# OSLL/slam-constructor

Hardware: AMD Instinct MI355X
Metric: pose-candidates*beams/sec (1080-beam scan, 2000^2 grid) (higher is better)
Workload: dtype f64; 1 GPU; cfg2: tinySLAM HC(dt 0.1, dr 0.1, failed-rounds 128), 1080 beams, 2000x2000 @0.05 m, occupancy cell; parallelism=1 gpu, ranks=1, includes_filter_and_upload=True, mode=default (canonical tree sum, device sincos; com~

## Files before the change

slam-constructor_amd/csrc/hc_chain.h:

```cpp
#pragma once

#include <cstdint>

#if defined(__HIPCC__)
#include <hip/hip_runtime.h>
#define HC_HD __host__ __device__ __forceinline__
#else
#define HC_HD inline
#endif

namespace slamhip {

constexpr int kHcMaxInst = 64;
constexpr int kHcDefaultInst = 42;
constexpr int kHcMaxSeg = 14;
constexpr int kHcShapes = 8;
constexpr int kHcSlots = 6 * kHcMaxInst + 1;

HC_HD double hc_bucket_rate(int b) { return 0.5 / (double)(1 << (kHcShapes - 1 - b)); }
HC_HD int hc_bucket_of_ratio(double num, double den) {
  int b = 0;
  for (int j = 0; j < kHcShapes - 1; ++j) b += (num > hc_bucket_rate(j) * 1.4142135623730951 * den) ? 1 : 0;
  return b;
}
HC_HD int hc_bucket_of(double p) { return hc_bucket_of_ratio(p, 1.0); }

struct HcInst {
  unsigned long long w[16];
};
static_assert(sizeof(HcInst) == 128, "HcInst layout");

HC_HD int hc_child(const HcInst &i, int out) {
  const unsigned long long v = out < 4 ? i.w[7] : i.w[8];
  return (int)(short)(unsigned short)(v >> (16 * (out & 3)));
}
HC_HD int hc_bp_inst(const HcInst &i) { return (int)(short)(unsigned short)(i.w[8] >> 48); }
HC_HD int hc_byte9(const HcInst &i, int k) { return (int)((i.w[9] >> (8 * k)) & 0xffull); }
HC_HD int hc_bp_cand(const HcInst &i) { return hc_byte9(i, 0); }
HC_HD unsigned hc_nfail(const HcInst &i) { return (unsigned)hc_byte9(i, 1); }
HC_HD unsigned hc_nfail_parent(const HcInst &i) { return (unsigned)hc_byte9(i, 2); }
HC_HD int hc_depth(const HcInst &i) { return hc_byte9(i, 3); }
HC_HD int hc_nseg(const HcInst &i) { return hc_byte9(i, 4); }
HC_HD bool hc_is_root(const HcInst &i) { return hc_byte9(i, 5) != 0; }
HC_HD unsigned hc_tail_fail(const HcInst &i) { return (unsigned)hc_byte9(i, 6); }
HC_HD int hc_parent(const HcInst &i) { return hc_byte9(i, 7) == 255 ? -1 : hc_byte9(i, 7); }
HC_HD unsigned hc_seg_fail(const HcInst &i, int k) {
  return (unsigned)(((k < 8 ? i.w[10] : i.w[11]) >> (8 * (k & 7))) & 0xffull);
}
HC_HD int hc_seg_out(const HcInst &i, int k) {
  return (int)(((k < 8 ? i.w[12] : i.w[13]) >> (8 * (k & 7))) & 0xffull);
}
inline void hc_set16(unsigned long long &w, int slot, int v) {
  w = (w & ~(0xffffull << (16 * slot))) | ((unsigned long long)(unsigned short)(short)v << (16 * slot));
}
inline void hc_set8(unsigned long long &w, int slot, unsigned v) {
  w = (w & ~(0xffull << (8 * slot))) | ((unsigned long long)(v & 0xff) << (8 * slot));
}
inline void hc_set_child(HcInst &i, int out, int v) { hc_set16(out < 4 ? i.w[7] : i.w[8], out & 3, v); }
inline void hc_set_bp_inst(HcInst &i, int v) { hc_set16(i.w[8], 3, v); }
inline void hc_set_byte9(HcInst &i, int k, unsigned v) { hc_set8(i.w[9], k, v); }
inline void hc_set_seg(HcInst &i, int k, unsigned fail, unsigned out) {
  hc_set8(k < 8 ? i.w[10] : i.w[11], k & 7, fail);
  hc_set8(k < 8 ? i.w[12] : i.w[13], k & 7, out);
}

struct HcShape {
  int n_inst;
  int pad[31];
  HcInst inst[kHcMaxInst];
};

struct HcState {
  double x, y, theta;
  double best_prob;
  double dt, dr;
  double recent_acc, recent_n;
  long long calls;
  long long evaluated;
  unsigned failed;
  int shape;
  int done;
  int first;
  int steps;
  int mode;
  int carry_cx, carry_cy;
  double carry_prob;
  unsigned long long best_hash;
  long long rescored;
};
static_assert(sizeof(HcState) == 136, "HcState layout");

HC_HD void hc_candidate(double x, double y, double theta, double dt, double dr, int c, double *ox, double *oy,
                        double *ot) {
  const double dir = (c % 2) ? -1.0 : 1.0;
  const double fcos = 1.0, fsin = 0.0;
  const int axis = c % 3;
  const double x0 = x + fcos * dir * dt, y0 = y + fsin * dir * dt;
  const double x1 = x + -fsin * dir * dt, y1 = y + fcos * dir * dt;
  const double t2 = theta + dir * dr;
  *ox = axis == 0 ? x0 : (axis == 1 ? x1 : x);
  *oy = axis == 0 ? y0 : (axis == 1 ? y1 : y);
  *ot = axis == 2 ? t2 : theta;
}

HC_HD bool hc_inert(double x, double y, double theta, double dt, double dr) {
  union U {
    double d;
    unsigned long long u;
  };
  U bx, by, bt;
  bx.d = x;
  by.d = y;
  bt.d = theta;
  bool same = true;
  for (int c = 0; c < 6; ++c) {
    U cx, cy, ct;
    hc_candidate(x, y, theta, dt, dr, c, &cx.d, &cy.d, &ct.d);
    same = same && cx.u == bx.u && cy.u == by.u && ct.u == bt.u;
  }
  return same;
}

HC_HD void hc_cert_beam(double px, double py, double sn, double cs, double theta_abs, double r_, double ca, double sa,
                        double scale, double inv_scale, double *t_t, double *t_r) {
  const double c = cs * ca - sn * sa;
  const double s_ = sn * ca + cs * sa;
  const double wx = px + r_ * c, wy = py + r_ * s_;
  const double qx = wx * inv_scale, qy = wy * inv_scale;
  const double fx = qx - __builtin_floor(qx), fy = qy - __builtin_floor(qy);
  const double mx = fx < 1.0 - fx ? fx : 1.0 - fx, my = fy < 1.0 - fy ? fy : 1.0 - fy;
  const double edge = (mx < my ? mx : my) * scale;
  const double ar = __builtin_fabs(r_);
  const double slack = (ar * (1.0 + theta_abs) + __builtin_fabs(wx) + __builtin_fabs(wy) + __builtin_fabs(px) +
                        __builtin_fabs(py) + 1.0) * 0x1p-44;
  const double avail = edge - slack;
  const bool ok = avail > 0.0;
  *t_t = ok ? avail * 0.99 : 0.0;
  *t_r = ok ? (ar > 0.0 ? avail / (1.5 * ar) : __builtin_inf()) : 0.0;
}

HC_HD double hc_pow_half(unsigned k) {
  union {
    unsigned long long u;
    double d;
  } v;
  v.u = (unsigned long long)(1023 - k) << 52;
  return v.d;
}

struct HcRound {
  double x, y, theta, dt, dr;
  unsigned failed;
};
HC_HD HcRound hc_round_of(const HcState &s, const HcInst &in) {
  HcRound r{s.x, s.y, s.theta, s.dt, s.dr, s.failed};
  const int nseg = hc_nseg(in);
  for (int k = 0; k < nseg; ++k) {
    const unsigned f = hc_seg_fail(in, k);
    const double h = hc_pow_half(f);
    r.dt *= h;
    r.dr *= h;
    r.failed += f;
    hc_candidate(r.x, r.y, r.theta, r.dt, r.dr, hc_seg_out(in, k) - 1, &r.x, &r.y, &r.theta);
  }
  const unsigned tf = hc_tail_fail(in);
  const double h = hc_pow_half(tf);
  r.dt *= h;
  r.dr *= h;
  r.failed += tf;
  return r;
}

HC_HD bool hc_trailing(unsigned failed_at_round, unsigned max_failed) { return failed_at_round >= max_failed; }

HC_HD int hc_round_outcome(double enter, const double *s, int n, double *run, int *nacc) {
  double b = enter;
  int out = 0, acc = 0;
  for (int c = 0; c < n; ++c)
    if (b < s[c]) {
      b = s[c];
      out = c + 1;
      ++acc;
    }
  *run = b;
  *nacc = acc;
  return out;
}

struct HcDecision {
  int out, nacc, last_acc;
  unsigned accmask;
  bool ambiguous;
};
HC_HD void hc_decide_one(HcDecision &d, double &b, unsigned long long &hb, int c, double s, unsigned long long h,
                         bool check) {
  union {
    double d;
    unsigned long long u;
  } sb{s}, bb{b};
  if (check && (h != hb || sb.u != bb.u)) {
    const double diff = s > b ? s - b : b - s;
    const double as = s < 0 ? -s : s, ab = b < 0 ? -b : b;
    if (diff <= (as > ab ? as : ab) * 9.094947017729282e-13) d.ambiguous = true;
  }
  if (b < s) {
    b = s;
    hb = h;
    d.out = c + 1;
    d.last_acc = c;
    d.accmask |= 1u << c;
    ++d.nacc;
  }
}
HC_HD HcDecision hc_round_decide(double enter, unsigned long long enter_hash, const double *dec,
                                 const unsigned long long *hash, int n, bool check) {
  HcDecision d{0, 0, -1, 0u, false};
  double b = enter;
  unsigned long long hb = enter_hash;
  for (int c = 0; c < n; ++c) hc_decide_one(d, b, hb, c, dec[c], hash[c], check);
  return d;
}

HC_HD HcRound hc_round_from(double x, double y, double theta, double dt, double dr, unsigned failed, const HcInst &in) {
  HcState s{};
  s.x = x;
  s.y = y;
  s.theta = theta;
  s.dt = dt;
  s.dr = dr;
  s.failed = failed;
  return hc_round_of(s, in);
}

struct HcNextCore {
  double x, y, theta, dt, dr;
  double recent_acc, recent_n;
  unsigned failed;
  int shape, done;
  long long batch_calls;
};
HC_HD HcNextCore hc_next_core(const HcState &prev, const HcInst &in, const HcRound &r, int out, unsigned max_failed) {
  HcNextCore n;
  n.x = r.x;
  n.y = r.y;
  n.theta = r.theta;
  n.dt = r.dt;
  n.dr = r.dr;
  n.failed = r.failed;
  if (out > 0) hc_candidate(r.x, r.y, r.theta, r.dt, r.dr, out - 1, &n.x, &n.y, &n.theta);
  const bool trailing = hc_trailing(r.failed, max_failed);
  n.done = trailing ? 1 : 0;
  if (!n.done && out == 0) {
    n.dt = r.dt * 0.5;
    n.dr = r.dr * 0.5;
    n.failed = r.failed + 1;
  }
  n.batch_calls = 6ll * hc_depth(in) + (trailing ? 1 : 6);
  const long long rounds_acc = (long long)hc_nseg(in) + (out > 0 ? 1 : 0);
  n.recent_acc = 0.5 * prev.recent_acc + (double)rounds_acc;
  n.recent_n = 0.5 * prev.recent_n + (double)n.batch_calls;
  n.shape = hc_bucket_of_ratio(n.recent_acc + 0.5, n.recent_n + 4.0);
  return n;
}

HC_HD void hc_advance(const HcState &prev, const HcInst &in, const HcRound &r, int out, double run, unsigned max_failed,
                      long long evaluated, HcState *next) {
  const HcNextCore c = hc_next_core(prev, in, r, out, max_failed);
  HcState n = prev;
  n.x = c.x;
  n.y = c.y;
  n.theta = c.theta;
  n.dt = c.dt;
  n.dr = c.dr;
  n.failed = c.failed;
  n.best_prob = run;
  n.done = c.done;
  n.calls = prev.calls + (prev.first ? 1 : 0) + c.batch_calls;
  n.evaluated = prev.evaluated + evaluated;
  n.first = 0;
  n.mode = 0;
  n.steps = prev.steps + 1;
  n.recent_acc = c.recent_acc;
  n.recent_n = c.recent_n;
  n.shape = c.shape;
  *next = n;
}

}
```

slam-constructor_amd/csrc/hc_resident.hip:

```cpp
#include <hip/hip_runtime.h>

#include "hc_chain_device.h"
#include "hc_resident_device.h"
#include "scan_assemble_device.h"
#include "score_device.h"

namespace slamhip {

namespace {
constexpr int kSumLanes = 256;
}

template <int H>
struct HcNextEntryT {
  double x, y, theta;
  double p[H][4];
  unsigned counts;
  unsigned flags;
};
static_assert(sizeof(HcNextEntryT<1>) == 64 && sizeof(HcNextEntryT<2>) == 96, "HcNextEntry layout");
static_assert(kHcMaxSeg + 1 <= 15, "HcNextEntry::counts: accepted rounds of a path in 4 bits");
static_assert(6 * kHcMaxInst + 6 < 4096, "HcNextEntry::counts: scorer calls of a path in 12 bits");
__device__ __forceinline__ unsigned hc_entry_counts(const HcNextCore &c, int rounds_acc) {
  return (c.failed & 0xffffu) | (((unsigned)c.batch_calls & 0xfffu) << 16) | (((unsigned)rounds_acc & 0xfu) << 28);
}

__device__ __forceinline__ void wave_min2(double &a, double &b) {
#define HCR_MIN_STEP(OFF)                              \
  {                                                    \
    const double oa = lane_xor_f64<OFF>(a), ob = lane_xor_f64<OFF>(b); \
    a = a < oa ? a : oa;                               \
    b = b < ob ? b : ob;                               \
  }
  HCR_MIN_STEP(32) HCR_MIN_STEP(16) HCR_MIN_STEP(8) HCR_MIN_STEP(4) HCR_MIN_STEP(2) HCR_MIN_STEP(1)
#undef HCR_MIN_STEP
}
__device__ __forceinline__ unsigned long long wave_xor_sum_u64(unsigned long long h) {
#define HCR_ADD_STEP(OFF)                                                                            \
  {                                                                                                  \
    const unsigned ol = lane_xor_u32<OFF>((unsigned)h), oh = lane_xor_u32<OFF>((unsigned)(h >> 32)); \
    h += ((unsigned long long)oh << 32) | ol;                                                        \
  }
  HCR_ADD_STEP(32) HCR_ADD_STEP(16) HCR_ADD_STEP(8) HCR_ADD_STEP(4) HCR_ADD_STEP(2) HCR_ADD_STEP(1)
#undef HCR_ADD_STEP
  return h;
}

constexpr int kSelRescore = -1;
constexpr int kSelFirst = -2;
constexpr int kSelStop = -3;

template <int MODEL, int NT, bool SEQ, bool BATCH, int G, bool WIN = false, bool PAIR = false, bool RAW = false>
__global__ __launch_bounds__(NT, 4) void k_hc_chain_resident(HcChainArgs a) {
  static_assert(!RAW || (!SEQ && !BATCH && !WIN && !PAIR), "RAW: the lone 1-cell chain in the default sum order only");
  constexpr int H = PAIR ? 2 : 1;
  constexpr int NTH = NT / H;
  constexpr bool CERT = !WIN;
  typedef HcNextEntryT<H> HcNextEntry;
  extern __shared__ double s_term[];
  __shared__ unsigned long long s_hash[kHcSlots + 7];
  __shared__ double s_sc[kHcSlots + 7];
  __shared__ HcInst s_mine[H][kHcShapes];
  __shared__ double s_cur[H][4];
  __shared__ int s_cur_go[H];
  __shared__ int s_sel;
  __shared__ int s_stop;
  __shared__ HcState s_st;
  __shared__ double s_part[H][4];
  __shared__ unsigned long long s_hpart[H][4];
  constexpr int kFpWaves = NTH / 64 > 4 ? NTH / 64 - 4 : 0;
  __shared__ unsigned long long s_hidle[kFpWaves > 0 ? kFpWaves : 1];
  __shared__ double s_cert[2][16];
  __shared__ int s_cert_end;
  const long long t_kernel_begin = SLAMHIP_STAMPS_ON(a.stamps != nullptr) ? (long long)wall_clock64() : 0ll;
  const int t = threadIdx.x, wave = t >> 6;
  const int half = PAIR ? (t >= NTH ? 1 : 0) : 0;
  const int tl = t - half * NTH, lwave = tl >> 6;
  const bool init_slot = blockIdx.x + 1 == gridDim.x;
  const int slot = init_slot ? kHcSlots - 1 : (PAIR ? 2 * (int)blockIdx.x + half : (int)blockIdx.x);
  const int inst_of_slot = slot / 6, cand = slot - 6 * inst_of_slot;
  const bool exists = init_slot ? half == 0 : slot < 6 * a.max_inst;
  HcResidentCtl *const rc = a.rctl + blockIdx.y;
  HcHostOut *const host = a.host + blockIdx.y;
  const unsigned fail_epoch_at_entry = __hip_atomic_load(&rc->fail_epoch, __ATOMIC_RELAXED, __HIP_MEMORY_SCOPE_AGENT);
#ifdef SLAMHIP_TESTING
  if (a.debug_mute && (int)blockIdx.x + 1 == a.debug_mute) return;
#endif
  MapViewCP map_p;
  ScanViewCP scan_p;
  {
    const __attribute__((address_space(4))) HcChainArgs *ap0 =
        (const __attribute__((address_space(4))) HcChainArgs *)__builtin_amdgcn_kernarg_segment_ptr();
    if (BATCH) {
      const __attribute__((address_space(4))) HcJobView *jv =
          (const __attribute__((address_space(4))) HcJobView *)(unsigned long long)(a.jobs + blockIdx.y);
      map_p = &jv->map;
      scan_p = &jv->scan;
    } else {
      map_p = &ap0->map;
      scan_p = &ap0->scan;
    }
  }
  const ScanView scan = load_view(scan_p);
  const int n = scan.n;
  double br = 0.0, bc = 0.0, bs = 0.0, bw = 0.0, bf = 0.0;
  if (!RAW && tl < n) {
    br = scan.range[tl];
    bc = scan.cos_a[tl];
    bs = scan.sin_a[tl];
    bw = scan.weight[tl];
    bf = scan.factor[tl];
  }
  const bool mine_here = lwave == 1 && (t & 63) < kHcShapes && !init_slot && exists;
  constexpr int kMineQ = (int)(sizeof(HcInst) / 16);
  static_assert(!RAW || kMineQ == 8, "RAW: the instance record in eight named registers");
  u32x4 mine0, mine1, mine2, mine3, mine4, mine5, mine6, mine7;
  ScanInFlight raw_first{0.0, 0.0, 0.0, 0.0, 1.0, 0}, raw_more{0.0, 0.0, 0.0, 0.0, 1.0, 0};
  HcInst first_in = {};
  const int n_last = n > 0 ? n - 1 : 0;
  const bool raw_more_wave = RAW && __builtin_amdgcn_readfirstlane(NTH + (t & ~63)) < n;
  if constexpr (RAW) {
    if (mine_here) {
      const u32x4 *src = reinterpret_cast<const u32x4 *>(&a.shapes[t & 63].inst[inst_of_slot]);
      mine0 = src[0];
      mine1 = src[1];
      mine2 = src[2];
      mine3 = src[3];
      mine4 = src[4];
      mine5 = src[5];
      mine6 = src[6];
      mine7 = src[7];
    }
    asm volatile("" ::: "memory");
    scan_assemble_issue(a.raw, tl < n ? tl : n_last, raw_first);
    if (raw_more_wave) scan_assemble_issue(a.raw, NTH + t < n ? NTH + t : n_last, raw_more);
    {
      const __attribute__((address_space(4))) HcInst *ip = (const __attribute__((address_space(4))) HcInst *)(
          unsigned long long)&a.shapes[a.shape0].inst[init_slot ? 0 : inst_of_slot];
#pragma unroll
      for (int q = 0; q < 14; ++q) first_in.w[q] = ip->w[q];
    }
  } else if (mine_here) {
    const uint4 *src = reinterpret_cast<const uint4 *>(&a.shapes[t & 63].inst[inst_of_slot]);
    uint4 *dst = reinterpret_cast<uint4 *>(&s_mine[half][t & 63]);
#pragma unroll
    for (int q = 0; q < kMineQ; ++q) dst[q] = src[q];
  }
  const bool ldsc = RAW || (!WIN && a.lds_consts != 0);
  const int n_more = n > NTH ? n - NTH : 0;
  double *const my_term = s_term + (PAIR ? half * a.scan.n : 0);
  double *const s_r = s_term + (PAIR ? 2 * a.scan.n : n) - NTH, *const s_ca = s_r + n_more, *const s_sa = s_ca + n_more;
  double *const s_w = s_sa + n_more, *const s_f = s_w + n_more;
  if (!RAW && ldsc) {
    for (int b = NTH + t; b < n; b += NT) {
      s_r[b] = scan.range[b];
      s_ca[b] = scan.cos_a[b];
      s_sa[b] = scan.sin_a[b];
    }
  }
  HcNextEntry *const s_tab = reinterpret_cast<HcNextEntry *>(s_term + a.tab_offset);
  if (!RAW && t == 0) s_stop = fail_epoch_at_entry == a.epoch ? 1 : 0;
  if (tl < 4 && exists) {
    HcGranule *g0 = (tl & 2) ? &rc->seq[tl & 1][slot] : &rc->gran[tl & 1][slot];
    gran_store(g0, 0.0, 0ull, 0u);
  }
  const bool verify = a.verify != 0;
  const bool stamp = SLAMHIP_STAMPS_ON(a.stamps && slot == 1 && tl == 0 && blockIdx.y == 0);
  [[maybe_unused]] const bool stamp_wave = SLAMHIP_STAMPS_ON(a.stamps && slot == 1 && tl < 64 && blockIdx.y == 0);
  if (stamp) a.stamps[6] = t_kernel_begin;
  HcGranule *const gran = &rc->gran[0][0];
  HcGranule *const gseq = &rc->seq[0][0];
  constexpr int kGranRow = kHcSlots + 7;

  if (t == 0) {
    HcState st{};
    const double *const inits = RAW ? nullptr : a.inits;
    st.x = inits ? inits[3 * blockIdx.y] : a.init[0];
    st.y = inits ? inits[3 * blockIdx.y + 1] : a.init[1];
    st.theta = inits ? inits[3 * blockIdx.y + 2] : a.init[2];
    st.dt = a.dt0;
    st.dr = a.dr0;
    st.shape = a.shape0;
    st.first = 1;
    st.carry_cx = st.carry_cy = -1;
    st.carry_prob = -1.0;
    s_st = st;
    s_sel = kSelFirst;
    s_cert_end = 0;
  }
  __syncthreads();
  if (!RAW && s_stop) return;
  if (lwave == 0) {
    const HcState &st = s_st;
    bool go = exists;
    double px = st.x, py = st.y, pth = st.theta;
    if (!init_slot && exists) {
      HcInst in;
#pragma unroll
      for (int q = 0; q < 14; ++q) in.w[q] = RAW ? first_in.w[q] : s_mine[half][st.shape].w[q];
      go = inst_of_slot < (int)((a.n_inst >> (8 * st.shape)) & 0xffull) &&
           (hc_is_root(in) || st.failed + hc_nfail_parent(in) < a.max_failed);
      if (go) {
        const HcRound r = hc_round_of(st, in);
        go = !(hc_trailing(r.failed, a.max_failed) && cand > 0);
        hc_candidate(r.x, r.y, r.theta, r.dt, r.dr, cand, &px, &py, &pth);
      }
    }
    double sn, cs;
    sincos(pth, &sn, &cs);
    if (tl == 0) {
      s_cur[half][0] = px;
      s_cur[half][1] = py;
      s_cur[half][2] = sn;
      s_cur[half][3] = cs;
      s_cur_go[half] = go ? 1 : 0;
    }
  }
  if constexpr (RAW) {
    const auto keep = [&](int b, const ScanPoint &p) __attribute__((always_inline)) {
      s_r[b] = p.range;
      s_ca[b] = p.cos_a;
      s_sa[b] = p.sin_a;
      s_w[b] = p.weight;
      s_f[b] = p.factor;
    };
    scan_assemble_wait(raw_first, raw_more);
    asm volatile("" ::"v"(mine0), "v"(mine1), "v"(mine2), "v"(mine3), "v"(mine4), "v"(mine5), "v"(mine6), "v"(mine7),
                 "v"(fail_epoch_at_entry));
    {
      ScanPoint p, pm;
      scan_assemble_finish(a.raw, raw_first, raw_more, p, pm);
      if (tl < n) {
        br = p.range;
        bc = p.cos_a;
        bs = p.sin_a;
        bw = p.weight;
        bf = p.factor;
      }
      if (NTH + t < n) keep(NTH + t, pm);
    }
    if (mine_here) {
      u32x4 *dst = reinterpret_cast<u32x4 *>(&s_mine[half][t & 63]);
      dst[0] = mine0;
      dst[1] = mine1;
      dst[2] = mine2;
      dst[3] = mine3;
      dst[4] = mine4;
      dst[5] = mine5;
      dst[6] = mine6;
      dst[7] = mine7;
    }
    if (t == 0) s_stop = fail_epoch_at_entry == a.epoch ? 1 : 0;
    for (int b = NTH + NT + t; b - (t & 63) < n; b += 2 * NT) {
      ScanInFlight f0{0.0, 0.0, 0.0, 0.0, 1.0, 0}, f1{0.0, 0.0, 0.0, 0.0, 1.0, 0};
      scan_assemble_issue(a.raw, b < n ? b : n_last, f0);
      scan_assemble_issue(a.raw, b + NT < n ? b + NT : n_last, f1);
      scan_assemble_wait(f0, f1);
      ScanPoint p0, p1;
      scan_assemble_finish(a.raw, f0, f1, p0, p1);
      if (b < n) keep(b, p0);
      if (b + NT < n) keep(b + NT, p1);
    }
  }
  __syncthreads();
  if (RAW && s_stop) return;

  auto write_scan_block = [&](int t, double *dst, int stride) __attribute__((always_inline)) {
    for (int q = t; q < stride; q += NT) {
      double r_ = 0.0, ca = 0.0, sa = 0.0, w = 0.0, f = 0.0;
      if (q < NT && q < n) {
        r_ = br;
        ca = bc;
        sa = bs;
        w = bw;
        f = bf;
      } else if (q < n) {
        r_ = s_r[q];
        ca = s_ca[q];
        sa = s_sa[q];
        w = s_w[q];
        f = s_f[q];
      }
      dst[q] = r_;
      dst[stride + q] = ca;
      dst[2 * stride + q] = sa;
      dst[3 * stride + q] = w;
      dst[4 * stride + q] = f;
    }
  };
  const int t_entry = t;
  for (int k = 0;; ++k) {
    const int pk = k & 1;
    int t = t_entry;
    asm volatile("" : "+v"(t));
    const int lane = t & 63;
    const int tl = PAIR ? t - half * NTH : t;
    const __attribute__((address_space(4))) HcChainArgs *ap =
        (const __attribute__((address_space(4))) HcChainArgs *)__builtin_amdgcn_kernarg_segment_ptr();
    asm volatile("" : "+s"(ap));
    MapViewCP mp = map_p;
    asm volatile("" : "+s"(mp));
    const MapView map = load_view(mp);
    if (stamp && k < 64) ap->stamps[8 * k + 0] = wall_clock64();
    const int sel = s_sel;
    if (sel == kSelStop) break;
    int go, mode = 0;
    double px, py, sn, cs;
    if (sel >= 0) {
      const HcNextEntry &e = s_tab[sel];
      const unsigned flags = e.flags;
      const bool cert_end = CERT && s_cert_end != 0;
      const int done = (int)((flags >> 3) & 1u) | (cert_end ? 1 : 0);
      go = (int)((flags >> (4 + half)) & 1u);
      px = e.p[half][0];
      py = e.p[half][1];
      sn = e.p[half][2];
      cs = e.p[half][3];
      if (wave == NT / 64 - 1 && lane < 1 + H) {
        if (lane == 0) {
          HcState &w = s_st;
          const unsigned counts = e.counts;
          const unsigned failed = counts & 0xffffu;
          const double half = hc_pow_half(failed - w.failed);
          w.x = e.x;
          w.y = e.y;
          w.theta = e.theta;
          w.dt = w.dt * half;
          w.dr = w.dr * half;
          w.recent_acc = 0.5 * w.recent_acc + (double)(counts >> 28);
          w.recent_n = 0.5 * w.recent_n + (double)((counts >> 16) & 0xfffu);
          w.failed = failed;
          w.shape = (int)(flags & 7u);
          w.done = done;
        } else {
          const int hh = lane - 1;
          s_cur[hh][0] = e.p[hh][0];
          s_cur[hh][1] = e.p[hh][1];
          s_cur[hh][2] = e.p[hh][2];
          s_cur[hh][3] = e.p[hh][3];
          s_cur_go[hh] = (int)((flags >> (4 + hh)) & 1u);
        }
      }
      long long tail_calls = 0;
      if (done && ((flags & 64u) || cert_end)) tail_calls = 6ll * (long long)(ap->max_failed - (e.counts & 0xffffu)) + 1ll;
      if (done && init_slot && tail_calls > 0 && ap->trace) {
        __syncthreads();
        HcTraceEntry *const trace = ap->trace + (size_t)blockIdx.y * (size_t)ap->trace_stride;
        const long long at0 = s_st.calls;
        const double best = s_st.best_prob, dt_e = s_st.dt, dr_e = s_st.dr;
        for (long long q = t; q < tail_calls; q += NT) {
          const double hlf = hc_pow_half((unsigned)(q / 6));
          HcTraceEntry te;
          hc_candidate(e.x, e.y, e.theta, dt_e * hlf, dr_e * hlf, (int)(q % 6), &te.x, &te.y, &te.theta);
          te.score = best;
          te.accepted = 0;
          te.pad = 0;
          if (at0 + q < ap->trace_cap) trace[at0 + q] = te;
          else host->error = 2;
        }
        __threadfence_system();
        __syncthreads();
      }
      if (done && init_slot && t == 0) {
        const HcState &w = s_st;
        const long long t_over = SLAMHIP_STAMPS_ON(ap->stamps != nullptr) ? (long long)wall_clock64() : 0ll;
        __threadfence_system();
        HcHostOut *h = host;
        h->pose[0] = e.x;
        h->pose[1] = e.y;
        h->pose[2] = e.theta;
        h->best_prob = w.best_prob;
        h->calls = w.calls + tail_calls;
        h->tail_calls = tail_calls;
        h->evaluated = w.evaluated;
        h->steps = w.steps;
        h->rescored = w.rescored;
        h->gm_cx = -1;
        h->gm_cy = -1;
        h->gm_prob = -1.0;
        __hip_atomic_store(&h->done_seq, ap->epoch, __ATOMIC_RELEASE, __HIP_MEMORY_SCOPE_SYSTEM);
        if (SLAMHIP_STAMPS_ON(ap->stamps != nullptr) && blockIdx.y == 0) {
          asm volatile("s_waitcnt vmcnt(0)" ::: "memory");
          ap->stamps[8 + 6] = t_over;
          ap->stamps[16 + 6] = wall_clock64();
        }
        if (ap->n_done) {
          __threadfence_system();
          const unsigned before = atomicAdd(ap->n_done, 1u);
          if (before + 1u == gridDim.y && ap->h_all_done)
            __hip_atomic_store(ap->h_all_done, ap->epoch, __ATOMIC_RELEASE, __HIP_MEMORY_SCOPE_SYSTEM);
        }
      }
      if constexpr (RAW) {
        if (done && init_slot && k == 1) write_scan_block(t, ap->raw.dst, (int)ap->raw.stride);
      }
      if (done) break;
    } else {
      if (sel == kSelRescore && init_slot) {
        if (wave == 0) {
          double sn_, cs_;
          sincos(s_st.theta, &sn_, &cs_);
          if (t == 0) {
            s_cur[0][0] = s_st.x;
            s_cur[0][1] = s_st.y;
            s_cur[0][2] = sn_;
            s_cur[0][3] = cs_;
            s_cur_go[0] = 1;
          }
        }
        __syncthreads();
      }
      go = s_cur_go[half];
      px = s_cur[half][0];
      py = s_cur[half][1];
      sn = s_cur[half][2];
      cs = s_cur[half][3];
      mode = sel == kSelRescore ? 1 : 0;
    }
    if (stamp && k < 64) ap->stamps[8 * k + 3] = wall_clock64();
    const unsigned tag = hc_tag(ap->tag_epoch, k);
    if (go) {
      if (WIN) {
        const double half_v = (ap->area[1] - ap->area[0]) / 2, half_h = (ap->area[3] - ap->area[2]) / 2;
        for (int b = tl; b < n; b += NTH) {
          double r_ = br, ca = bc, sa = bs, w = bw, f = bf;
          if (b != tl) {
            r_ = scan.range[b];
            ca = scan.cos_a[b];
            sa = scan.sin_a[b];
            w = scan.weight[b];
            f = scan.factor[b];
          }
          const double c = cs * ca - sn * sa;
          const double s = sn * ca + cs * sa;
          const double ox = px + r_ * c, oy = py + r_ * s;
          my_term[b] = window_probability<MODEL>(map, ap->oie, ap->oope, half_v, half_h, ox, oy) * w * f;
        }
      } else {
        constexpr int UNR = NTH == 256 ? 5 : 4;
        for (int base = tl; base < n; base += UNR * NTH) {
          double4 cell[UNR];
          double w_[UNR], f_[UNR];
  #pragma unroll
          for (int j = 0; j < UNR; ++j) {
            const int b = base + j * NTH;
            w_[j] = 0.0;
            f_[j] = 0.0;
            cell[j] = make_double4(0.0, 0.0, 0.0, 0.0);
            if ((base - lane) + j * NTH >= n) continue;
            const int bc_ = b < n ? b : n - 1;
            double r_ = br, ca = bc, sa = bs;
            w_[j] = bw;
            f_[j] = bf;
            if (j > 0 || base != tl) {
              r_ = ldsc ? s_r[bc_] : scan.range[bc_];
              ca = ldsc ? s_ca[bc_] : scan.cos_a[bc_];
              sa = ldsc ? s_sa[bc_] : scan.sin_a[bc_];
              w_[j] = RAW ? s_w[bc_] : scan.weight[bc_];
              f_[j] = RAW ? s_f[bc_] : scan.factor[bc_];
            }
            cell[j] = beam_cell<MODEL>(map, px, py, sn, cs, r_, ca, sa);
          }
  #pragma unroll
          for (int j = 0; j < UNR; ++j) {
            const int b = base + j * NTH;
            if (b < n) my_term[b] = cell_probability<MODEL>(ap->oie, cell[j]) * w_[j] * f_[j];
          }
        }
      }
    }
    double cert_t = 0.0, cert_r = 0.0;
    const bool cert_here = CERT && init_slot && half == 0 && sel >= 0 && !go && ap->inert_tail > 1;
    if (cert_here) {
      const double theta_abs = __builtin_fabs(s_tab[sel].theta);
      double tt = __builtin_inf(), tr = __builtin_inf();
      for (int b = tl; b < n; b += NTH) {
        double r_ = br, ca = bc, sa = bs;
        if (b != tl) {
          r_ = ldsc ? s_r[b] : scan.range[b];
          ca = ldsc ? s_ca[b] : scan.cos_a[b];
          sa = ldsc ? s_sa[b] : scan.sin_a[b];
        }
        double t1, t2;
        hc_cert_beam(px, py, sn, cs, theta_abs, r_, ca, sa, map.scale, map.inv_scale, &t1, &t2);
        tt = tt < t1 ? tt : t1;
        tr = tr < t2 ? tr : t2;
      }
      wave_min2(tt, tr);
      if (lane == 0) {
        s_cert[0][lwave] = tt;
        s_cert[1][lwave] = tr;
      }
    }
    __syncthreads();
    if (cert_here && tl < 64) {
      double tt = tl < NTH / 64 ? s_cert[0][tl] : __builtin_inf(), tr = tl < NTH / 64 ? s_cert[1][tl] : __builtin_inf();
      wave_min2(tt, tr);
      cert_t = tt;
      cert_r = tr;
    }
    if (stamp && k < 64) ap->stamps[8 * k + 4] = wall_clock64();
#ifdef SLAMHIP_TESTING
    if (ap->debug_mute < 0) {
      const int dm = -ap->debug_mute, every = (dm >> 16) & 15, phase = (dm >> 20) & 15, who = dm & 0xffff;
      if ((who == 0xffff ? init_slot : (int)blockIdx.x + 1 == who) && every > 0 && k % every == phase)
        for (int q = 0; q < 5; ++q) __builtin_amdgcn_s_sleep(16);
    }
#endif
    if (go) {
      if (SEQ) {
        if (tl == 0) {
          double acc = 0.0;
          int b = 0;
          for (; b + 8 <= n; b += 8) {
            const double t0 = my_term[b], t1 = my_term[b + 1], t2 = my_term[b + 2], t3 = my_term[b + 3];
            const double t4 = my_term[b + 4], t5 = my_term[b + 5], t6 = my_term[b + 6], t7 = my_term[b + 7];
            acc = acc + t0;
            acc = acc + t1;
            acc = acc + t2;
            acc = acc + t3;
            acc = acc + t4;
            acc = acc + t5;
            acc = acc + t6;
            acc = acc + t7;
          }
          for (; b < n; ++b) acc = acc + my_term[b];
          gran_store(&gran[pk * kGranRow + slot], (scan.tot_w == 0.0) ? __builtin_nan("") : acc / scan.tot_w, 0ull, tag);
        }
      } else if (tl < kSumLanes) {
        double acc = 0.0;
        unsigned long long h = 0ull;
        unsigned k_lo = (2u * (unsigned)tl + 1u) * 0x9E3779B1u, k_hi = (2u * (unsigned)tl + 1u) * 0x85EBCA6Bu;
        for (int b = tl; b < n; b += kSumLanes) {
          const double term = my_term[b];
          acc = acc + term;
          if (kFpWaves == 0 && verify) {
            h += term_fingerprint(term, k_lo, k_hi);
            k_lo += 2u * kSumLanes * 0x9E3779B1u;
            k_hi += 2u * kSumLanes * 0x85EBCA6Bu;
          }
        }
        if (kFpWaves == 0) wave_xor_sum_with(acc, h);
        else acc = wave_xor_sum(acc);
        if (lane == 0) {
          s_part[half][lwave] = acc;
          if (kFpWaves == 0) s_hpart[half][lwave] = h;
        }
      } else if (kFpWaves > 0 && verify) {
        const int w = lwave - kSumLanes / 64;
        const int per = (n + kFpWaves - 1) / kFpWaves;
        const int b_end = (w + 1) * per < n ? (w + 1) * per : n;
        unsigned long long h = 0ull;
        for (int b = w * per + lane; b < b_end; b += 64)
          h += term_fingerprint(my_term[b], (2u * (unsigned)b + 1u) * 0x9E3779B1u, (2u * (unsigned)b + 1u) * 0x85EBCA6Bu);
        h = wave_xor_sum_u64(h);
        if (lane == 0) s_hidle[w] = h;
      }
    }
    __syncthreads();
    if (go) {
      if (!SEQ) {
        if (tl == 0) {
          const double total = (s_part[half][0] + s_part[half][1]) + (s_part[half][2] + s_part[half][3]);
          unsigned long long fp = 0ull;
          if (verify) {
            unsigned long long h = 0ull;
            if (kFpWaves == 0) h = s_hpart[half][0] + s_hpart[half][1] + s_hpart[half][2] + s_hpart[half][3];
#pragma unroll
            for (int w = 0; w < kFpWaves; ++w) h += s_hidle[w];
            fp = fold_fingerprint48(h);
          }
          gran_store(&gran[pk * kGranRow + slot], (scan.tot_w == 0.0) ? __builtin_nan("") : total / scan.tot_w, fp, tag);
        }
        if (verify && mode && tl == 64) {
          double acc = 0.0;
          for (int b = 0; b < n; ++b) acc = acc + my_term[b];
          gran_store(&gseq[pk * kGranRow + slot], (scan.tot_w == 0.0) ? __builtin_nan("") : acc / scan.tot_w, 0ull, tag);
        }
      }
      if (stamp && k < 64) ap->stamps[8 * k + 5] = wall_clock64();
    } else if (tl == 0 && exists) {
      gran_store(&gran[pk * kGranRow + slot], cert_here ? cert_t : 0.0,
                 cert_here ? (unsigned long long)__double_as_longlong(cert_r) >> 16 : 0ull, tag);
      if (verify && mode) gran_store(&gseq[pk * kGranRow + slot], 0.0, 0ull, tag);
    }
    if constexpr (RAW) {
      if (init_slot && k == 1) write_scan_block(t, ap->raw.dst, (int)ap->raw.stride);
    }

    if (wave != 0) {
      {
        const HcState &sp = s_st;
        const int shape = sp.shape;
        const int n_inst = (int)((ap->n_inst >> (8 * shape)) & 0xffull);
        const unsigned max_failed = ap->max_failed;
        for (int e = t - 64; e < 7 * n_inst; e += NT - 64) {
          const int ti = e / 7, out = e - 7 * ti;
          HcInst in;
          {
            const unsigned long long *src = &ap->shapes[shape].inst[ti].w[0];
#pragma unroll
            for (int q = 0; q < 14; ++q) in.w[q] = src[q];
          }
          if (!(hc_is_root(in) || sp.failed + hc_nfail_parent(in) < max_failed)) continue;
          const bool trailing = hc_trailing(sp.failed + hc_nfail(in), max_failed);
          if (trailing ? out > 1 : hc_child(in, out) >= 0) continue;
          const HcRound r = hc_round_of(sp, in);
          const HcNextCore c = hc_next_core(sp, in, r, out, max_failed);
          HcNextEntry &w = s_tab[e];
          w.x = c.x;
          w.y = c.y;
          w.theta = c.theta;
          w.counts = hc_entry_counts(c, hc_nseg(in) + (out > 0 ? 1 : 0));
          const bool inert = !c.done && ap->inert_tail && hc_inert(c.x, c.y, c.theta, c.dt, c.dr);
          unsigned flags = (unsigned)c.shape | (c.done || inert ? 8u : 0u) | (inert ? 64u : 0u);
#pragma unroll
          for (int hh = 0; hh < H; ++hh) {
            const int slot_h = PAIR ? 2 * (int)blockIdx.x + hh : slot;
            const int inst_h = slot_h / 6, cand_h = slot_h - 6 * inst_h;
            bool go = !c.done && !inert && !init_slot && slot_h < 6 * ap->max_inst;
            double px_ = c.x, py_ = c.y, pth_ = c.theta;
            if (go) {
              HcInst mine;
#pragma unroll
              for (int q = 0; q < 14; ++q) mine.w[q] = s_mine[hh][c.shape].w[q];
              go = inst_h < (int)((ap->n_inst >> (8 * c.shape)) & 0xffull) &&
                   (hc_is_root(mine) || c.failed + hc_nfail_parent(mine) < max_failed);
              if (go) {
                const HcRound r2 = hc_round_from(c.x, c.y, c.theta, c.dt, c.dr, c.failed, mine);
                go = !(hc_trailing(r2.failed, max_failed) && cand_h > 0);
                hc_candidate(r2.x, r2.y, r2.theta, r2.dt, r2.dr, cand_h, &px_, &py_, &pth_);
              }
            }
            double sn_ = 0.0, cs_ = 1.0;
            if (go || (CERT && init_slot && hh == 0 && ap->inert_tail > 1)) sincos(pth_, &sn_, &cs_);
            w.p[hh][0] = px_;
            w.p[hh][1] = py_;
            w.p[hh][2] = sn_;
            w.p[hh][3] = cs_;
            flags |= go ? (16u << hh) : 0u;
          }
          w.flags = flags;
        }
      }
    } else {
      const HcState &sp = s_st;
      const int n_inst = (int)((ap->n_inst >> (8 * sp.shape)) & 0xffull);
      HcInst me;
      {
        const unsigned long long *src = &ap->shapes[sp.shape].inst[lane].w[0];
#pragma unroll
        for (int q = 0; q < 14; ++q) me.w[q] = src[q];
      }
      const bool active = lane < n_inst;
      const bool reach = active && (hc_is_root(me) || sp.failed + hc_nfail_parent(me) < ap->max_failed);
      const bool trailing = reach && hc_trailing(sp.failed + hc_nfail(me), ap->max_failed);
      const int bpi = hc_bp_inst(me);
      const int bp_slot = (!active || bpi < 0) ? -1 : 6 * bpi + hc_bp_cand(me);
      const bool base_here = sp.first || sp.mode == 1;
      const int n_grid = 6 * ap->max_inst;
      const bool rescored = !SEQ && verify && sp.mode == 1;
      bool failed = false;
      unsigned sweep_polls = 0u;
      int missing_first = 0;
      {
        const HcGranule *g0 = gran + pk * kGranRow;
        unsigned spins = 0;
        for (;;) {
          u32x4 g[G];
          const HcGranule *gp[G];
          bool ok = true;
#pragma unroll
          for (int q = 0; q < G; ++q) {
            const int i = lane + 64 * q;
            gp[q] = g0 + (i < n_grid ? i : kHcSlots - 1);
          }
          gran_fetch(g, gp);
#pragma unroll
          for (int q = 0; q < G; ++q) {
            const int i = lane + 64 * q;
            const int j = i < n_grid ? i : kHcSlots - 1;
            const bool here = gran_tag(g[q]) == tag;
            ok = ok && here;
            if (here) {
              s_sc[j] = gran_score(g[q]);
              s_hash[j] = gran_hash(g[q]);
            }
            if (SLAMHIP_STAMPS_ON(stamp_wave) && spins == 0u) missing_first += __popcll(__ballot(!here && i <= n_grid));
          }
          if (__all(ok)) break;
          ++spins;
          if (BATCH) __builtin_amdgcn_s_sleep(8);
          if ((spins & 31u) == 0u) {
            const bool gone = __hip_atomic_load(&rc->fail_epoch, __ATOMIC_RELAXED, __HIP_MEMORY_SCOPE_AGENT) == ap->epoch;
            if (gone || spins > ap->spin_limit) {
              failed = true;
              break;
            }
          }
        }
        sweep_polls = spins + 1u;
      }
      if (stamp && k < 64) ap->stamps[8 * k + 1] = wall_clock64();
      if (failed || k + 1 >= kHcResidentMaxSteps) {
        if (lane == 0) {
          __hip_atomic_store(&rc->fail_epoch, ap->epoch, __ATOMIC_RELAXED, __HIP_MEMORY_SCOPE_AGENT);
          __hip_atomic_store(&host->error, failed ? 4 : 5, __ATOMIC_RELAXED, __HIP_MEMORY_SCOPE_SYSTEM);
          __threadfence_system();
          __hip_atomic_store(&host->done_seq, ap->epoch, __ATOMIC_RELEASE, __HIP_MEMORY_SCOPE_SYSTEM);
          s_sel = kSelStop;
        }
      } else {
        double root_prob = sp.first ? s_sc[kHcSlots - 1] : sp.best_prob;
        double s6[6];
#pragma unroll
        for (int c = 0; c < 6; ++c) s6[c] = s_sc[6 * lane + c];
        const double enter = bp_slot < 0 ? root_prob : s_sc[bp_slot];
        double run = enter;
        int out = 0;
        unsigned accmask = 0u;
        bool ambiguous = false;
        unsigned long long run_hash = 0ull;
        if (!SEQ && verify) {
          const unsigned long long root_hash = base_here ? s_hash[kHcSlots - 1] : sp.best_hash;
          unsigned long long hb = bp_slot < 0 ? root_hash : s_hash[bp_slot];
          unsigned long long h6[6];
#pragma unroll
          for (int c = 0; c < 6; ++c) h6[c] = s_hash[6 * lane + c];
          if (!rescored) {
            int amb = 0;
#pragma unroll
            for (int c = 0; c < 6; ++c) {
              const double s = s6[c];
              const double diff = __builtin_fabs(s - run);
              const double as = __builtin_fabs(s), ab = __builtin_fabs(run);
              const int live = (c == 0) | (int)!trailing;
              const int close = (int)(diff <= (as > ab ? as : ab) * 9.094947017729282e-13);
              amb |= live & close & ((int)(h6[c] != hb) | (int)(__double_as_longlong(s) != __double_as_longlong(run)));
              const bool acc = (live & (int)(run < s)) != 0;
              run = acc ? s : run;
              hb = acc ? h6[c] : hb;
              out = acc ? c + 1 : out;
              accmask |= acc ? 1u << c : 0u;
            }
            ambiguous = amb != 0;
          } else {
            const HcGranule *q0 = gseq + pk * kGranRow;
            double bdec = 0.0;
#pragma unroll 1
            for (int c = -1; c < 6; ++c) {
              const int j = c < 0 ? (bp_slot < 0 ? kHcSlots - 1 : bp_slot) : (active ? 6 * lane + c : kHcSlots - 1);
              double sd = 0.0;
              for (unsigned spins = 0;; ++spins) {
                u32x4 g[1];
                const HcGranule *gp[1] = {q0 + j};
                gran_fetch(g, gp);
                sd = gran_score(g[0]);
                if (__all(gran_tag(g[0]) == tag) || spins > ap->spin_limit) break;
              }
              if (c < 0) {
                bdec = sd;
                continue;
              }
              const bool acc = active && (c == 0 || !trailing) && bdec < sd;
              bdec = acc ? sd : bdec;
              run = acc ? s_sc[6 * lane + c] : run;
              hb = acc ? s_hash[6 * lane + c] : hb;
              out = acc ? c + 1 : out;
              accmask |= acc ? 1u << c : 0u;
            }
          }
          run_hash = hb;
        } else {
#pragma unroll
          for (int c = 0; c < 6; ++c)
            if ((c == 0 || !trailing) && run < s6[c]) {
              run = s6[c];
              out = c + 1;
              accmask |= 1u << c;
            }
        }
        bool valid = reach;
#pragma unroll
        for (int o = 0; o < 7; ++o) {
          const unsigned long long has = __ballot(reach && out == o);
          valid = valid && (me.w[o] & ~has) == 0ull;
        }
        const bool terminal = valid && (trailing || hc_child(me, out) < 0);
        const unsigned long long tmask = __ballot(terminal);
        const int tl = tmask ? __ffsll((long long)tmask) - 1 : 0;
        if (stamp && k < 64) ap->stamps[8 * k + 7] = wall_clock64();
        const bool dirty = !SEQ && verify && sp.mode == 0 && __ballot(valid && ambiguous) != 0ull;
        const int out_t = bcast_i(out, tl);
        const double run_t = bcast(run, tl);
        const int depth_t = bcast_i(hc_depth(me), tl);
        const bool trailing_t = bcast_i(trailing ? 1 : 0, tl) != 0;
        const unsigned long long run_hash_t = (unsigned long long)bcast_ll((long long)run_hash, tl);
        if (init_slot && ap->trace && !dirty) {
          HcTraceEntry *const trace = ap->trace + (size_t)blockIdx.y * (size_t)ap->trace_stride;
          const long long base = sp.calls + (sp.first ? 1 : 0);
          if (sp.first && lane == 0 && ap->trace_cap > 0) {
            HcTraceEntry e{sp.x, sp.y, sp.theta, root_prob, 1, 0};
            trace[0] = e;
          }
          if (valid) {
            const HcRound rr = hc_round_of(sp, me);
            const int nc = trailing ? 1 : 6;
            for (int c = 0; c < nc; ++c) {
              HcTraceEntry e;
              hc_candidate(rr.x, rr.y, rr.theta, rr.dt, rr.dr, c, &e.x, &e.y, &e.theta);
              e.score = s_sc[6 * lane + c];
              e.accepted = (accmask >> c) & 1u;
              e.pad = 0;
              const long long at = base + 6ll * hc_depth(me) + c;
              if (at < ap->trace_cap) trace[at] = e;
              else host->error = 2;
            }
          }
        }
        bool cert_end = false;
        if (CERT && ap->inert_tail > 1 && !sp.first && sp.mode == 0 && !dirty && tmask != 0ull) {
          const int nseg_t = bcast_i(hc_nseg(me), tl), nfail_t = bcast_i((int)hc_nfail(me), tl);
          const unsigned failed_next = sp.failed + (unsigned)nfail_t + 1u;
          if (nseg_t == 0 && out_t == 0 && !trailing_t && failed_next < ap->max_failed) {
            const double hlf = hc_pow_half((unsigned)nfail_t + 1u);
            const double t_t = s_sc[kHcSlots - 1];
            const double t_r = __longlong_as_double((long long)(s_hash[kHcSlots - 1] << 16));
            cert_end = sp.dt * hlf < t_t && sp.dr * hlf < t_r;
          }
        }
        if (stamp && k < 64) ap->stamps[8 * k + 2] = wall_clock64();
        if (stamp && k >= 3 && k < 64) ap->stamps[8 * k + 6] = (long long)sweep_polls | ((long long)missing_first << 32);
        if (lane == 0) {
          s_cert_end = cert_end ? 1 : 0;
          HcState &w = s_st;
          if (tmask == 0ull) {
            if (init_slot) {
              __hip_atomic_store(&host->error, 1, __ATOMIC_RELAXED, __HIP_MEMORY_SCOPE_SYSTEM);
              __threadfence_system();
              __hip_atomic_store(&host->done_seq, ap->epoch, __ATOMIC_RELEASE, __HIP_MEMORY_SCOPE_SYSTEM);
            }
            s_sel = kSelStop;
          } else if (!dirty) {
            w.best_prob = run_t;
            w.calls = sp.calls + (sp.first ? 1 : 0) + 6ll * depth_t + (trailing_t ? 1 : 6);
            w.evaluated = sp.evaluated + 6ll * n_inst + (sp.first ? 1 : 0);
            w.first = 0;
            w.mode = 0;
            w.steps = sp.steps + 1;
            if (!SEQ && verify) w.best_hash = run_hash_t;
            s_sel = 7 * tl + out_t;
          } else {
            w.mode = 1;
            w.steps = sp.steps + 1;
            w.evaluated = sp.evaluated + 6ll * n_inst + 1;
            w.rescored = sp.rescored + 1;
            s_sel = kSelRescore;
          }
        }
      }
    }
    __syncthreads();
  }
}

size_t hc_resident_tab_offset(int nt, int n_beams, int lds_consts, bool pair) {
  const size_t n = (size_t)(n_beams > 0 ? n_beams : 1);
  const size_t nth = (size_t)(pair ? nt / 2 : nt);
  const size_t more = lds_consts && n > nth ? n - nth : 0;
  return (pair ? 2 : 1) * n + (lds_consts > 1 ? 5 : 3) * more;
}
size_t hc_resident_lds_bytes(int nt, int n_beams, int lds_consts, int max_inst, bool pair) {
  return sizeof(double) * hc_resident_tab_offset(nt, n_beams, lds_consts, pair) +
         (pair ? sizeof(HcNextEntryT<2>) : sizeof(HcNextEntryT<1>)) * 7 * (size_t)max_inst;
}

// ... 57 lines not shown
```

Baseline: 14.22 billion pose-candidates*beams/s.

## Fuse beam-term reduction into the scoring loop via register accumulation

For 256-thread-per-pose chains in the default sum order, each lane now accumulates its beam probability terms in registers and reduces them across the wave with lane shuffles. Terms are no longer written to shared memory and re-read, except in verify mode. One block-wide barrier is skipped when no certificate is computed. A beam-to-lane permutation helper is added so the tree-sum order can be kept for larger groups, which adds index arithmetic and more complex fingerprint and reduction code paths.

```diff
diff --git a/slam-constructor_amd/csrc/hc_chain.h b/slam-constructor_amd/csrc/hc_chain.h
--- a/slam-constructor_amd/csrc/hc_chain.h
+++ b/slam-constructor_amd/csrc/hc_chain.h
@@ -138,6 +138,12 @@
   *t_t = ok ? avail * 0.99 : 0.0;
   *t_r = ok ? (ar > 0.0 ? avail / (1.5 * ar) : __builtin_inf()) : 0.0;
 }
+
+HC_HD int hc_partial_of(int tl, int nth) {
+  const int T = nth / 256, w = tl >> 6, l = tl & 63;
+  return 64 * (w / T) + T * (l / T) + w % T;
+}
+HC_HD int hc_beam_of(int tl, int nth) { return hc_partial_of(tl, nth) + 256 * ((tl & 63) % (nth / 256)); }
 
 HC_HD double hc_pow_half(unsigned k) {
   union {
diff --git a/slam-constructor_amd/csrc/hc_resident.hip b/slam-constructor_amd/csrc/hc_resident.hip
--- a/slam-constructor_amd/csrc/hc_resident.hip
+++ b/slam-constructor_amd/csrc/hc_resident.hip
@@ -46,6 +46,63 @@
   return h;
 }
 
+template <int T, int J>
+__device__ __forceinline__ double group_bcast_f64(double v) {
+  static_assert((T == 2 || T == 4) && J >= 0 && J < T, "pairs or quads");
+  constexpr int kCtrl = T == 4 ? J * 0x55 : (J == 0 ? 0xA0 : 0xF5);
+  const unsigned long long b = (unsigned long long)__double_as_longlong(v);
+  const int lo = __builtin_amdgcn_update_dpp((int)(unsigned)b, (int)(unsigned)b, kCtrl, 0xF, 0xF, false);
+  const int hi = __builtin_amdgcn_update_dpp((int)(unsigned)(b >> 32), (int)(unsigned)(b >> 32), kCtrl, 0xF, 0xF, false);
+  return __longlong_as_double((long long)(((unsigned long long)(unsigned)hi << 32) | (unsigned)lo));
+}
+template <int T>
+__device__ __forceinline__ double group_chain_add(double acc, double term) {
+  if constexpr (T == 1) return acc + term;
+  if constexpr (T == 2) return (acc + group_bcast_f64<2, 0>(term)) + group_bcast_f64<2, 1>(term);
+  if constexpr (T == 4)
+    return (((acc + group_bcast_f64<4, 0>(term)) + group_bcast_f64<4, 1>(term)) + group_bcast_f64<4, 2>(term)) +
+           group_bcast_f64<4, 3>(term);
+}
+template <int OFF>
+__device__ __forceinline__ void lane_xor_add_u64(unsigned long long &h) {
+  const unsigned ol = lane_xor_u32<OFF>((unsigned)h), oh = lane_xor_u32<OFF>((unsigned)(h >> 32));
+  h += ((unsigned long long)oh << 32) | ol;
+}
+template <int T, bool WITH_H>
+__device__ __forceinline__ void lane_sum_wave(double &v, unsigned long long &h) {
+  if constexpr (WITH_H) {
+    if constexpr (T == 4) lane_xor_add_u64<2>(h);
+    if constexpr (T >= 2) lane_xor_add_u64<1>(h);
+    wave_xor_step_with<32>(v, h);
+    wave_xor_step_with<16>(v, h);
+    wave_xor_step_with<8>(v, h);
+    wave_xor_step_with<4>(v, h);
+    if constexpr (T <= 2) wave_xor_step_with<2>(v, h);
+    if constexpr (T == 1) wave_xor_step_with<1>(v, h);
+  } else {
+    v = v + lane_xor_f64<32>(v);
+    v = v + lane_xor_f64<16>(v);
+    v = v + lane_xor_f64<8>(v);
+    v = v + lane_xor_f64<4>(v);
+    if constexpr (T <= 2) v = v + lane_xor_f64<2>(v);
+    if constexpr (T == 1) v = v + lane_xor_f64<1>(v);
+  }
+}
+template <int T, bool WITH_H>
+__device__ __forceinline__ void lane_sum_combine(double &v, unsigned long long &h) {
+  if constexpr (WITH_H) {
+    if constexpr (T == 4) wave_xor_step_with<2>(v, h);
+    if constexpr (T >= 2) wave_xor_step_with<1>(v, h);
+    wave_xor_step_with<T>(v, h);
+    wave_xor_step_with<2 * T>(v, h);
+  } else {
+    if constexpr (T == 4) v = v + lane_xor_f64<2>(v);
+    if constexpr (T >= 2) v = v + lane_xor_f64<1>(v);
+    v = v + lane_xor_f64<T>(v);
+    v = v + lane_xor_f64<2 * T>(v);
+  }
+}
+
 constexpr int kSelRescore = -1;
 constexpr int kSelFirst = -2;
 constexpr int kSelStop = -3;
@@ -56,6 +113,10 @@
   constexpr int H = PAIR ? 2 : 1;
   constexpr int NTH = NT / H;
   constexpr bool CERT = !WIN;
+  constexpr bool LANE = !SEQ && !WIN && NTH == 256;
+  constexpr int T = NTH / 256;
+  constexpr int kParts = LANE ? NTH / 64 : 4;
+  static_assert(!LANE || (T == 1 || T == 2 || T == 4), "LANE: 256, 512 or 1024 threads per pose");
   typedef HcNextEntryT<H> HcNextEntry;
   extern __shared__ double s_term[];
   __shared__ unsigned long long s_hash[kHcSlots + 7];
@@ -66,9 +127,9 @@
   __shared__ int s_sel;
   __shared__ int s_stop;
   __shared__ HcState s_st;
-  __shared__ double s_part[H][4];
-  __shared__ unsigned long long s_hpart[H][4];
-  constexpr int kFpWaves = NTH / 64 > 4 ? NTH / 64 - 4 : 0;
+  __shared__ double s_part[H][kParts];
+  __shared__ unsigned long long s_hpart[H][kParts];
+  constexpr int kFpWaves = !LANE && NTH / 64 > 4 ? NTH / 64 - 4 : 0;
   __shared__ unsigned long long s_hidle[kFpWaves > 0 ? kFpWaves : 1];
   __shared__ double s_cert[2][16];
   __shared__ int s_cert_end;
@@ -76,6 +137,8 @@
   const int t = threadIdx.x, wave = t >> 6;
   const int half = PAIR ? (t >= NTH ? 1 : 0) : 0;
   const int tl = t - half * NTH, lwave = tl >> 6;
+  const int b0 = LANE ? hc_beam_of(tl, NTH) : tl;
+  const int bw0 = LANE ? hc_beam_of(tl & ~63, NTH) : (tl & ~63);
   const bool init_slot = blockIdx.x + 1 == gridDim.x;
   const int slot = init_slot ? kHcSlots - 1 : (PAIR ? 2 * (int)blockIdx.x + half : (int)blockIdx.x);
   const int inst_of_slot = slot / 6, cand = slot - 6 * inst_of_slot;
@@ -104,12 +167,12 @@
   const ScanView scan = load_view(scan_p);
   const int n = scan.n;
   double br = 0.0, bc = 0.0, bs = 0.0, bw = 0.0, bf = 0.0;
-  if (!RAW && tl < n) {
-    br = scan.range[tl];
-    bc = scan.cos_a[tl];
-    bs = scan.sin_a[tl];
-    bw = scan.weight[tl];
-    bf = scan.factor[tl];
+  if (!RAW && b0 < n) {
+    br = scan.range[b0];
+    bc = scan.cos_a[b0];
+    bs = scan.sin_a[b0];
+    bw = scan.weight[b0];
+    bf = scan.factor[b0];
   }
   const bool mine_here = lwave == 1 && (t & 63) < kHcShapes && !init_slot && exists;
   constexpr int kMineQ = (int)(sizeof(HcInst) / 16);
@@ -118,7 +181,7 @@
   ScanInFlight raw_first{0.0, 0.0, 0.0, 0.0, 1.0, 0}, raw_more{0.0, 0.0, 0.0, 0.0, 1.0, 0};
   HcInst first_in = {};
   const int n_last = n > 0 ? n - 1 : 0;
-  const bool raw_more_wave = RAW && __builtin_amdgcn_readfirstlane(NTH + (t & ~63)) < n;
+  const bool raw_more_wave = RAW && __builtin_amdgcn_readfirstlane(NTH + bw0) < n;
   if constexpr (RAW) {
     if (mine_here) {
       const u32x4 *src = reinterpret_cast<const u32x4 *>(&a.shapes[t & 63].inst[inst_of_slot]);
@@ -132,8 +195,8 @@
       mine7 = src[7];
     }
     asm volatile("" ::: "memory");
-    scan_assemble_issue(a.raw, tl < n ? tl : n_last, raw_first);
-    if (raw_more_wave) scan_assemble_issue(a.raw, NTH + t < n ? NTH + t : n_last, raw_more);
+    scan_assemble_issue(a.raw, b0 < n ? b0 : n_last, raw_first);
+    if (raw_more_wave) scan_assemble_issue(a.raw, NTH + b0 < n ? NTH + b0 : n_last, raw_more);
     {
       const __attribute__((address_space(4))) HcInst *ip = (const __attribute__((address_space(4))) HcInst *)(
           unsigned long long)&a.shapes[a.shape0].inst[init_slot ? 0 : inst_of_slot];
@@ -230,14 +293,14 @@
     {
       ScanPoint p, pm;
       scan_assemble_finish(a.raw, raw_first, raw_more, p, pm);
-      if (tl < n) {
+      if (b0 < n) {
         br = p.range;
         bc = p.cos_a;
         bs = p.sin_a;
         bw = p.weight;
         bf = p.factor;
       }
-      if (NTH + t < n) keep(NTH + t, pm);
+      if (NTH + b0 < n) keep(NTH + b0, pm);
     }
     if (mine_here) {
       u32x4 *dst = reinterpret_cast<u32x4 *>(&s_mine[half][t & 63]);
@@ -251,7 +314,7 @@
       dst[7] = mine7;
     }
     if (t == 0) s_stop = fail_epoch_at_entry == a.epoch ? 1 : 0;
-    for (int b = NTH + NT + t; b - (t & 63) < n; b += 2 * NT) {
+    for (int b = NTH + NT + b0; b - (b0 - bw0) < n; b += 2 * NT) {
       ScanInFlight f0{0.0, 0.0, 0.0, 0.0, 1.0, 0}, f1{0.0, 0.0, 0.0, 0.0, 1.0, 0};
       scan_assemble_issue(a.raw, b < n ? b : n_last, f0);
       scan_assemble_issue(a.raw, b + NT < n ? b + NT : n_last, f1);
@@ -266,7 +329,7 @@
   if (RAW && s_stop) return;
 
   auto write_scan_block = [&](int t, double *dst, int stride) __attribute__((always_inline)) {
-    for (int q = t; q < stride; q += NT) {
+    for (int q = LANE ? hc_beam_of(t, NT) : t; q < stride; q = q < NT ? NT + t : q + NT) {
       double r_ = 0.0, ca = 0.0, sa = 0.0, w = 0.0, f = 0.0;
       if (q < NT && q < n) {
         r_ = br;
@@ -295,6 +358,8 @@
     asm volatile("" : "+v"(t));
     const int lane = t & 63;
     const int tl = PAIR ? t - half * NTH : t;
+    const int bw0 = LANE ? hc_beam_of(__builtin_amdgcn_readfirstlane(tl) & ~63, NTH) : __builtin_amdgcn_readfirstlane(tl) & ~63;
+    const int b0 = bw0 + (LANE ? hc_beam_of(lane, NTH) : lane);
     const __attribute__((address_space(4))) HcChainArgs *ap =
         (const __attribute__((address_space(4))) HcChainArgs *)__builtin_amdgcn_kernarg_segment_ptr();
     asm volatile("" : "+s"(ap));
@@ -306,6 +371,8 @@
     if (sel == kSelStop) break;
     int go, mode = 0;
     double px, py, sn, cs;
+    [[maybe_unused]] double acc = 0.0;
+    [[maybe_unused]] unsigned long long hsum = 0ull;
     if (sel >= 0) {
       const HcNextEntry &e = s_tab[sel];
       const unsigned flags = e.flags;
@@ -438,7 +505,8 @@
         }
       } else {
         constexpr int UNR = NTH == 256 ? 5 : 4;
-        for (int base = tl; base < n; base += UNR * NTH) {
+        for (int wb = bw0; wb < n; wb += UNR * NTH) {
+          const int base = wb + (b0 - bw0);
           double4 cell[UNR];
           double w_[UNR], f_[UNR];
   #pragma unroll
@@ -447,12 +515,12 @@
             w_[j] = 0.0;
             f_[j] = 0.0;
             cell[j] = make_double4(0.0, 0.0, 0.0, 0.0);
-            if ((base - lane) + j * NTH >= n) continue;
+            if (wb + j * NTH >= n) continue;
             const int bc_ = b < n ? b : n - 1;
             double r_ = br, ca = bc, sa = bs;
             w_[j] = bw;
             f_[j] = bf;
-            if (j > 0 || base != tl) {
+            if (j > 0 || wb != bw0) {
               r_ = ldsc ? s_r[bc_] : scan.range[bc_];
               ca = ldsc ? s_ca[bc_] : scan.cos_a[bc_];
               sa = ldsc ? s_sa[bc_] : scan.sin_a[bc_];
@@ -461,22 +529,44 @@
             }
             cell[j] = beam_cell<MODEL>(map, px, py, sn, cs, r_, ca, sa);
           }
+          double term[UNR];
   #pragma unroll
           for (int j = 0; j < UNR; ++j) {
             const int b = base + j * NTH;
-            if (b < n) my_term[b] = cell_probability<MODEL>(ap->oie, cell[j]) * w_[j] * f_[j];
+            term[j] = 0.0;
+            if (b < n) term[j] = cell_probability<MODEL>(ap->oie, cell[j]) * w_[j] * f_[j];
+            if ((!LANE || mode) && b < n) my_term[b] = term[j];
+          }
+          if constexpr (LANE) {
+            if (stamp && k < 64 && wb == bw0) ap->stamps[8 * k + 4] = wall_clock64();
+  #pragma unroll
+            for (int j = 0; j < UNR; ++j) {
+              if (wb + j * NTH >= n) continue;
+              acc = group_chain_add<T>(acc, term[j]);
+              const unsigned kb = 2u * (unsigned)(base + j * NTH) + 1u;
+              if (verify) hsum += term_fingerprint(term[j], kb * 0x9E3779B1u, kb * 0x85EBCA6Bu);
+            }
+          }
+        }
+        if constexpr (LANE) {
+          if (verify) lane_sum_wave<T, true>(acc, hsum);
+          else lane_sum_wave<T, false>(acc, hsum);
+          if (lane == 0) {
+            s_part[half][tl >> 6] = acc;
+            if (verify) s_hpart[half][tl >> 6] = hsum;
           }
         }
       }
     }
     double cert_t = 0.0, cert_r = 0.0;
-    const bool cert_here = CERT && init_slot && half == 0 && sel >= 0 && !go && ap->inert_tail > 1;
+    const bool cert_wg = CERT && init_slot && sel >= 0 && ap->inert_tail > 1;
+    const bool cert_here = cert_wg && half == 0 && !go;
     if (cert_here) {
       const double theta_abs = __builtin_fabs(s_tab[sel].theta);
       double tt = __builtin_inf(), tr = __builtin_inf();
-      for (int b = tl; b < n; b += NTH) {
+      for (int b = b0; b < n; b += NTH) {
         double r_ = br, ca = bc, sa = bs;
-        if (b != tl) {
+        if (b != b0) {
           r_ = ldsc ? s_r[b] : scan.range[b];
           ca = ldsc ? s_ca[b] : scan.cos_a[b];
           sa = ldsc ? s_sa[b] : scan.sin_a[b];
@@ -492,14 +582,14 @@
         s_cert[1][lwave] = tr;
       }
     }
-    __syncthreads();
+    if (!LANE || cert_wg) __syncthreads();
     if (cert_here && tl < 64) {
       double tt = tl < NTH / 64 ? s_cert[0][tl] : __builtin_inf(), tr = tl < NTH / 64 ? s_cert[1][tl] : __builtin_inf();
       wave_min2(tt, tr);
       cert_t = tt;
       cert_r = tr;
     }
-    if (stamp && k < 64) ap->stamps[8 * k + 4] = wall_clock64();
+    if (!LANE && stamp && k < 64) ap->stamps[8 * k + 4] = wall_clock64();
 #ifdef SLAMHIP_TESTING
     if (ap->debug_mute < 0) {
       const int dm = -ap->debug_mute, every = (dm >> 16) & 15, phase = (dm >> 20) & 15, who = dm & 0xffff;
@@ -507,7 +597,7 @@
         for (int q = 0; q < 5; ++q) __builtin_amdgcn_s_sleep(16);
     }
 #endif
-    if (go) {
+    if (!LANE && go) {
       if (SEQ) {
         if (tl == 0) {
           double acc = 0.0;
@@ -559,7 +649,21 @@
     }
     __syncthreads();
     if (go) {
-      if (!SEQ) {
+      if constexpr (LANE) {
+        if (tl < 64) {
+          double total = lane < kParts ? s_part[half][lane] : 0.0;
+          unsigned long long h = 0ull;
+          if (verify) {
+            h = lane < kParts ? s_hpart[half][lane] : 0ull;
+            lane_sum_combine<T, true>(total, h);
+          } else {
+            lane_sum_combine<T, false>(total, h);
+          }
+          if (lane == 0)
+            gran_store(&gran[pk * kGranRow + slot], (scan.tot_w == 0.0) ? __builtin_nan("") : total / scan.tot_w,
+                       verify ? fold_fingerprint48(h) : 0ull, tag);
+        }
+      } else if (!SEQ) {
         if (tl == 0) {
           const double total = (s_part[half][0] + s_part[half][1]) + (s_part[half][2] + s_part[half][3]);
           unsigned long long fp = 0ull;
@@ -572,6 +676,8 @@
           }
           gran_store(&gran[pk * kGranRow + slot], (scan.tot_w == 0.0) ? __builtin_nan("") : total / scan.tot_w, fp, tag);
         }
+      }
+      if (!SEQ) {
         if (verify && mode && tl == 64) {
           double acc = 0.0;
           for (int b = 0; b < n; ++b) acc = acc + my_term[b];
```

Result: faster. 14.37 billion pose-candidates*beams/s (median of 6 runs) (+1.1%).
